# daniabib/ComfyUI_ProPainter_Nodes

Measured on NVIDIA H100. Metric: inpainted frames/sec at 640x360, 80-frame subvideo, higher is better.
Workload: dtype f16

## Files before the change

comfyui_propainter_nodes_b200/csrc/conv_epilogue.cuh:

```cuda
#pragma once
#include "conv_igemm.cuh"
#include "wgmma_ops.cuh"

namespace ppconv {

template <int ACT>
__device__ __forceinline__ void act16_t(float (&v)[16], float slope) {
#pragma unroll
  for (int i = 0; i < 16; ++i) {
    if (ACT == PP_ACT_RELU) v[i] = fmaxf(v[i], 0.f);
    else if (ACT == PP_ACT_LRELU) v[i] = v[i] > 0.f ? v[i] : v[i] * slope;
    else if (ACT == PP_ACT_SIGMOID) v[i] = ppx::sigmoidf_(v[i]);
    else if (ACT == PP_ACT_TANH) v[i] = tanhf(v[i]);
    else if (ACT == PP_ACT_GELU) v[i] = ppx::gelu_erf(v[i]);
  }
}
__device__ __forceinline__ void act16(float (&v)[16], int act, float slope) {
  switch (act) {
    case PP_ACT_RELU: act16_t<PP_ACT_RELU>(v, slope); break;
    case PP_ACT_LRELU: act16_t<PP_ACT_LRELU>(v, slope); break;
    case PP_ACT_SIGMOID: act16_t<PP_ACT_SIGMOID>(v, slope); break;
    case PP_ACT_TANH: act16_t<PP_ACT_TANH>(v, slope); break;
    case PP_ACT_GELU: act16_t<PP_ACT_GELU>(v, slope); break;
    default: break;
// ... 3 lines not shown
__device__ __forceinline__ void load16(const __half* src, int nvalid, bool vec, float (&r)[16]) {
  if (vec && nvalid == 16) {
    const uint4 a = reinterpret_cast<const uint4*>(src)[0], b = reinterpret_cast<const uint4*>(src)[1];
    const __half2* ha = reinterpret_cast<const __half2*>(&a);
    const __half2* hb = reinterpret_cast<const __half2*>(&b);
#pragma unroll
    for (int i = 0; i < 4; ++i) {
      const float2 fa = __half22float2(ha[i]), fb = __half22float2(hb[i]);
      r[2 * i] = fa.x; r[2 * i + 1] = fa.y; r[8 + 2 * i] = fb.x; r[8 + 2 * i + 1] = fb.y;
    }
  } else {
#pragma unroll
    for (int i = 0; i < 16; ++i) r[i] = i < nvalid ? __half2float(src[i]) : 0.f;
  }
}
__device__ __forceinline__ void store16(__half* dst, int nvalid, bool vec, const float (&v)[16]) {
  if (vec && nvalid == 16) {
    __align__(16) __half2 h[8];
#pragma unroll
    for (int i = 0; i < 8; ++i) h[i] = __floats2half2_rn(v[2 * i], v[2 * i + 1]);
    reinterpret_cast<uint4*>(dst)[0] = reinterpret_cast<uint4*>(h)[0];
    reinterpret_cast<uint4*>(dst)[1] = reinterpret_cast<uint4*>(h)[1];
  } else {
#pragma unroll
    for (int i = 0; i < 16; ++i)
      if (i < nvalid) dst[i] = __float2half_rn(v[i]);
  }
}

__device__ __forceinline__ void unpack16(const uint4& a, const uint4& b, float (&r)[16]) {
  const __half2* ha = reinterpret_cast<const __half2*>(&a);
  const __half2* hb = reinterpret_cast<const __half2*>(&b);
#pragma unroll
  for (int i = 0; i < 4; ++i) {
    const float2 fa = __half22float2(ha[i]), fb = __half22float2(hb[i]);
    r[2 * i] = fa.x; r[2 * i + 1] = fa.y; r[8 + 2 * i] = fb.x; r[8 + 2 * i + 1] = fb.y;
  }
// ... 16 lines not shown
    if (ng0 >= half_c) s0 = p.aux0 + mrow * p.aux0_cstride + p.aux0_coff + (ng0 - half_c);
  } else {
    s0 = p.aux0 + mrow * p.aux0_cstride + p.aux0_coff + ng0;
    s1 = p.aux1 + mrow * p.aux1_cstride + p.aux1_coff + ng0;
  }
  if (s0 == nullptr) return;
  x.have = true;
  x.a0[0] = reinterpret_cast<const uint4*>(s0)[0];
  x.a0[1] = reinterpret_cast<const uint4*>(s0)[1];
  if (s1 != nullptr) {
    x.a1[0] = reinterpret_cast<const uint4*>(s1)[0];
    x.a1[1] = reinterpret_cast<const uint4*>(s1)[1];
  }
}

__device__ __forceinline__ void conv_epilogue16(const PPConvParams& p, const uint32_t (&raw)[16], long long mrow, int g,
                                                int ng0, int epi, bool vec, const EpiAux* pre = nullptr,
                                                uint4* sm0 = nullptr, uint4* sm1 = nullptr) {
    const int nvalid = min(16, p.Cout_g - ng0);
    float v[16];
#pragma unroll
    for (int i = 0; i < 16; ++i) v[i] = __uint_as_float(raw[i]);
    if (p.bias != nullptr) {
      const float* bp = p.bias + g * p.Cout_g + ng0;
      if (vec && nvalid == 16) {
#pragma unroll
        for (int i = 0; i < 4; ++i) {
          const float4 b4 = __ldg(reinterpret_cast<const float4*>(bp) + i);
          v[4 * i] += b4.x; v[4 * i + 1] += b4.y; v[4 * i + 2] += b4.z; v[4 * i + 3] += b4.w;
        }
// ... 24 lines not shown
#pragma unroll
          for (int i = 0; i < 4; ++i)
            reinterpret_cast<float4*>(dst)[i] = make_float4(v[4 * i], v[4 * i + 1], v[4 * i + 2], v[4 * i + 3]);
        } else {
#pragma unroll
          for (int i = 0; i < 16; ++i)
            if (i < nvalid) dst[i] = v[i];
        }
      } else if (sm0 != nullptr) {
        __align__(16) __half2 h[8];
#pragma unroll
        for (int i = 0; i < 8; ++i) h[i] = __floats2half2_rn(v[2 * i], v[2 * i + 1]);
        *sm0 = reinterpret_cast<uint4*>(h)[0];
        *sm1 = reinterpret_cast<uint4*>(h)[1];
      } else {
        store16(reinterpret_cast<__half*>(p.out) + o, nvalid, vec, v);
      }
    } else if (epi == PP_EPI_GRU_ZR) {
      const int half_c = p.Cout_g >> 1;
      act16_t<PP_ACT_SIGMOID>(v, 0.f);
      if (ng0 < half_c) {
        store16(reinterpret_cast<__half*>(p.out) + mrow * p.out_cstride + p.out_coff + ng0, nvalid, vec, v);
      } else {
        const int c = ng0 - half_c;
        float h[16];
        if (pre != nullptr && pre->have) unpack16(pre->a0[0], pre->a0[1], h);
        else load16(p.aux0 + mrow * p.aux0_cstride + p.aux0_coff + c, nvalid, vec, h);
#pragma unroll
        for (int i = 0; i < 16; ++i) v[i] *= h[i];
        store16(p.out2 + mrow * p.out2_cstride + p.out2_coff + c, nvalid, vec, v);
      }
    } else {
      float h[16], z[16];
      if (pre != nullptr && pre->have) {
        unpack16(pre->a0[0], pre->a0[1], h);
        unpack16(pre->a1[0], pre->a1[1], z);
      } else {
        load16(p.aux0 + mrow * p.aux0_cstride + p.aux0_coff + ng0, nvalid, vec, h);
        load16(p.aux1 + mrow * p.aux1_cstride + p.aux1_coff + ng0, nvalid, vec, z);
      }
      act16_t<PP_ACT_TANH>(v, 0.f);
#pragma unroll
      for (int i = 0; i < 16; ++i) v[i] = (1.f - z[i]) * h[i] + z[i] * v[i];
      store16(reinterpret_cast<__half*>(p.out) + mrow * p.out_cstride + p.out_coff + ng0, nvalid, vec, v);
    }
}

constexpr int STG_LD = 40;
constexpr int STG_BYTES = 64 * STG_LD * 4;

template <int N, class Emit>
__device__ __forceinline__ void drain_acc(const float (&acc)[N / 2], float* stg, int t128, int bar_id, Emit&& emit) {
  const int wrow = 16 * (t128 >> 5) + ((t128 & 31) >> 2), wcol = 2 * (t128 & 3);
#pragma unroll 1
  for (int c0 = 0; c0 < N; c0 += 32) {
#pragma unroll
    for (int cc = 0; cc < N; cc += 32) {
      if (cc == c0) {
#pragma unroll
// ... 1 lines not shown
          if (cc + 8 * j < N) {
            const int i = (cc / 8 + j) * 4;
            *reinterpret_cast<float2*>(stg + wrow * STG_LD + 8 * j + wcol) = make_float2(acc[i], acc[i + 1]);
            *reinterpret_cast<float2*>(stg + (wrow + 8) * STG_LD + 8 * j + wcol) = make_float2(acc[i + 2], acc[i + 3]);
          }
        }
      }
    }
    ppx::named_bar(bar_id, 128);
    const int c = c0 + 16 * (t128 & 1);
    if (c < N) emit(stg + (t128 >> 1) * STG_LD + 16 * (t128 & 1), t128 >> 1, c);
    ppx::named_bar(bar_id, 128);
  }
}

__device__ __forceinline__ void epilogue_from_stage(const PPConvParams& p, const float* src, long long mrow, int g, int ng0,
                                                    uint4* sm0, uint4* sm1) {
  uint32_t raw[16];
#pragma unroll
  for (int i = 0; i < 16; i += 4) {
    const float4 v = *reinterpret_cast<const float4*>(src + i);
    raw[i] = __float_as_uint(v.x); raw[i + 1] = __float_as_uint(v.y);
    raw[i + 2] = __float_as_uint(v.z); raw[i + 3] = __float_as_uint(v.w);
  }
  conv_epilogue16(p, raw, mrow, g, ng0, p.epi, p.vec_ok != 0, nullptr, sm0, sm1);
}

template <int V>
struct IntC { static constexpr int value = V; };
template <int MAX_N, class F>
__device__ __forceinline__ void with_tile_width(int bn, F&& f) {
  switch (bn) {
    case 16: f(IntC<16>{}); break;
    case 32: f(IntC<32>{}); break;
    case 48: f(IntC<48>{}); break;
    case 64: f(IntC<64>{}); break;
    case 80: f(IntC<80>{}); break;
    case 96: f(IntC<96>{}); break;
    case 112: f(IntC<112>{}); break;
    case 128: f(IntC<128>{}); break;
// ... 21 lines not shown
```

comfyui_propainter_nodes_b200/csrc/conv_halo.cu:

```cuda
#include <cuda.h>
#include <stdlib.h>
#include <string.h>

#include <memory>

#include "conv_epilogue.cuh"
#include "conv_igemm.cuh"
#include "dcn_sample.cuh"

namespace {

constexpr int NUM_THREADS = 384;
constexpr int NUM_EPI_THREADS = 256;
constexpr int WARP_A = 8, WARP_B = 9;
constexpr int UPS_THREADS = 416, UPS_INTERP_THREADS = 128;
constexpr int UPS_WARP_B = 12;
constexpr int MAX_SA = 4, MAX_SB = 8;
constexpr int SMEM_BUDGET = 186 * 1024;

struct HaloParams {
  PPConvParams c;
  CUtensorMap tmap[4];
  int MT;
  int BW, BH;
  int tiles_x, tiles_y, n_tiles;
  int a_stage_bytes, b_stage_bytes, SA, SB;
  int tps;
  int chunks;
  int flat;
  int n_img;
  int sub_bytes;
  int ups;
  int LH, LW;
  int LBW, LBH;
  int l_stage_bytes;
  int debug;
  int tstore;
  int out_stage_bytes;
  CUtensorMap tmap_out;
};

__device__ __forceinline__ void tma_load_4d(uint32_t dst, const void* tmap, int c0, int c1, int c2, int c3, uint64_t* bar) {
  asm volatile(
      "cp.async.bulk.tensor.4d.shared::cluster.global.mbarrier::complete_tx::bytes [%0], [%1, {%3, %4, %5, %6}], [%2];" ::"r"(dst),
      "l"(tmap), "r"(ppx::smem_u32(bar)), "r"(c0), "r"(c1), "r"(c2), "r"(c3)
      : "memory");
// ... 11 lines not shown
  TileCoord t;
  t.n_idx = tile % h.n_tiles;
  int r = tile / h.n_tiles;
  t.tx = r % h.tiles_x; r /= h.tiles_x;
  t.ty = r % h.tiles_y; r /= h.tiles_y;
  t.img = r % h.n_img;
  t.g = r / h.n_img;
  return t;
}

struct Ring {
  int s;
  uint32_t ph;
};

__host__ __device__ constexpr int halo_max_tps(int bn) { return 128 / bn > 1 ? 128 / bn : 1; }

template <int BN, int MB>
__device__ __forceinline__ void halo_tap(float (&acc)[MB][BN / 2], uint64_t (&adesc)[MB], uint64_t& bdesc, uint32_t& accum,
                                         int& kx, int kw, uint32_t step_x, uint32_t step_row, uint32_t tap16) {
#pragma unroll
  for (int k = 0; k < 4; ++k)
#pragma unroll
    for (int b = 0; b < MB; ++b) ppx::wgmma_f16<BN>(acc[b], adesc[b] + 2 * k, bdesc + 2 * k, (accum | k) != 0 ? 1u : 0u);
  accum = 1u;
  bdesc += tap16;
  const uint32_t step = ++kx == kw ? step_row : step_x;
  if (kx == kw) kx = 0;
#pragma unroll
  for (int b = 0; b < MB; ++b) adesc[b] += step;
}
// ... 9 lines not shown
    wgmma_commit();
  } else {
    if constexpr (NT > 1) {
      if (tn < NT) {
        halo_tap_group<BN, MB, NT - 1>(tn, acc, adesc, bdesc, accum, kx, kw, step_x, step_row, tap16);
        return;
      }
    }
    wgmma_fence();
#pragma unroll
    for (int tt = 0; tt < NT; ++tt) halo_tap<BN, MB>(acc, adesc, bdesc, accum, kx, kw, step_x, step_row, tap16);
    wgmma_commit();
  }
}

template <int BN, int MB, int NT>
__device__ __forceinline__ void halo_tile(const HaloParams& h, int tile, uint8_t* smem, uint8_t* smem_b, int SA, int SB,
                                          int a_stage_bytes, int b_stage_bytes, uint64_t* a_full, uint64_t* a_empty,
                                          uint64_t* b_full, uint64_t* b_empty, Ring& ra, Ring& rb, float* stg,
                                          uint8_t* stg_out, int wg, int t128) {
  using namespace ppx;
  const PPConvParams& p = h.c;
  const int taps = p.kh * p.kw;
  const TileCoord t = decode_tile(h, tile);
  const int n0 = t.n_idx * p.BN;
  const int bnt = min(p.BN, p.Cout_g_pad - n0);
  const uint32_t sbo = h.flat ? 1024u : (uint32_t)h.BW * 128;
  const uint32_t step_x = (uint32_t)p.dw * 8;
  const uint32_t step_row = (uint32_t)(p.dh * h.BW - (p.kw - 1) * p.dw) * 8;
  const uint32_t tap16 = (uint32_t)p.BN * 8;
  const int kw = p.kw;
  uint32_t aoff[MB];
#pragma unroll
  for (int b = 0; b < MB; ++b) aoff[b] = MB == 2 ? wg * h.sub_bytes + b * 8 * sbo : wg * 8 * sbo;
  float acc[MB][BN / 2];
  uint32_t accum = 0;
  int pend_a = -1, pend_b = -1;
  for (int c = 0; c < h.chunks; ++c) {
    mbar_wait(&a_full[ra.s], ra.ph);
    uint64_t adesc[MB];
#pragma unroll
    for (int b = 0; b < MB; ++b) adesc[b] = gmma_desc_sw128_kmajor(smem_u32(smem + ra.s * a_stage_bytes) + aoff[b], sbo);
    int kx = 0;
    for (int tap0 = 0; tap0 < taps; tap0 += h.tps) {
      mbar_wait(&b_full[rb.s], rb.ph);
      const uint64_t bdesc = gmma_desc_sw128_kmajor(smem_u32(smem_b + rb.s * b_stage_bytes));
      halo_tap_group<BN, MB, NT>(min(h.tps, taps - tap0), acc, adesc, bdesc, accum, kx, kw, step_x, step_row, tap16);
      wgmma_wait<1>();
      if (pend_b >= 0) mbar_arrive(&b_empty[pend_b]);
      if (pend_a >= 0) mbar_arrive(&a_empty[pend_a]);
      pend_b = rb.s;
      pend_a = tap0 + h.tps >= taps ? ra.s : -1;
      if (++rb.s == SB) { rb.s = 0; rb.ph ^= 1; }
    }
    if (++ra.s == SA) { ra.s = 0; ra.ph ^= 1; }
  }
  wgmma_wait<0>();
#pragma unroll
  for (int b = 0; b < MB; ++b) wgmma_fence_acc(acc[b]);
  if (pend_b >= 0) mbar_arrive(&b_empty[pend_b]);
  if (pend_a >= 0) mbar_arrive(&a_empty[pend_a]);

  const bool skip = (h.debug & 1) != 0;
  const int bar_id = 2 + (MB == 2 ? wg : 0), bar_n = MB == 2 ? 128 : 256;
  const bool issuer = t128 == 0 && (MB == 2 || wg == 0);
  uint8_t* so = h.tstore ? stg_out + (MB == 2 ? wg : 0) * h.out_stage_bytes : nullptr;
  if (so != nullptr) {
    if (issuer) asm volatile("cp.async.bulk.wait_group.read 0;" ::: "memory");
    named_bar(bar_id, bar_n);
  }
#pragma unroll
  for (int b = 0; b < MB; ++b) {
    const int sub = MB == 2 ? wg : 0, rbase = MB == 2 ? 64 * b : 64 * wg;
    ppconv::drain_acc<BN>(acc[b], stg, t128, 4 + wg, [&](const float* src, int r64, int cc) {
      const int r = rbase + r64;
      bool mvalid;
      long long mrow;
      if (h.flat) {
        mrow = ((long long)t.tx * h.MT + sub) * 128 + r;
        mvalid = mrow < p.M_total;
      } else {
        const int oy = t.ty * 16 + (r >> 3), ox = t.tx * (8 * h.MT) + 8 * sub + (r & 7);
        mvalid = oy < p.OH && ox < p.OW;
        mrow = ((long long)t.img * p.OH + oy) * p.OW + ox;
      }
      if (!mvalid || skip || cc >= bnt || n0 + cc >= p.Cout_g) return;
      if (so != nullptr) {
        auto slot = [&](int u) {
          const int unit = ((cc & 63) >> 3) + u;
          return reinterpret_cast<uint4*>(so + (cc >> 6) * 16384 + r * 128 + ((unit ^ (r & 7)) << 4));
        };
        ppconv::epilogue_from_stage(p, src, mrow, t.g, n0 + cc, slot(0), slot(1));
      } else {
        ppconv::epilogue_from_stage(p, src, mrow, t.g, n0 + cc, nullptr, nullptr);
      }
    });
  }
  if (so != nullptr) {
    fence_proxy_async();
    named_bar(bar_id, bar_n);
    if (issuer && !skip) {
      const int row0 = (int)(((long long)t.tx * h.MT + (MB == 2 ? wg : 0)) * 128);
      for (int pnl = 0; pnl * 64 < bnt; ++pnl)
        tma_store_2d(&h.tmap_out, smem_u32(so + pnl * 16384), n0 + pnl * 64, row0);
      asm volatile("cp.async.bulk.commit_group;" ::: "memory");
    }
  }
}

template <class F>
__device__ __forceinline__ void with_tile_shape(int mt, int bn, F&& f) {
  if (mt == 2) ppconv::with_tile_width<128>(bn, [&](auto n) { f(n, ppconv::IntC<2>{}); });
  else ppconv::with_tile_width<256>(bn, [&](auto n) { f(n, ppconv::IntC<1>{}); });
}

template <bool UPS>
__global__ void __launch_bounds__(UPS ? UPS_THREADS : NUM_THREADS, 1) conv_halo_kernel(const __grid_constant__ HaloParams h) {
  using namespace ppx;
  const PPConvParams& p = h.c;
  extern __shared__ uint8_t smem_raw[];
  const uint32_t raw_addr = smem_u32(smem_raw);
  uint8_t* smem = smem_raw + (((raw_addr + 1023u) & ~1023u) - raw_addr);
  uint8_t* smem_b = smem + h.SA * h.a_stage_bytes;
  uint64_t* a_full = reinterpret_cast<uint64_t*>(smem_b + h.SB * h.b_stage_bytes);
  uint64_t* a_empty = a_full + MAX_SA;
  uint64_t* b_full = a_empty + MAX_SA;
  uint64_t* b_empty = b_full + MAX_SB;
  uint64_t* l_full = b_empty + MAX_SB;
  uint64_t* l_empty = l_full + 2;
  uint8_t* stg_out = smem_b + h.SB * h.b_stage_bytes + 2048;
  float* acc_stg = reinterpret_cast<float*>(smem_b + h.SB * h.b_stage_bytes + 1024 + (UPS ? 2 * h.l_stage_bytes : 0) +
                                            (h.tstore ? 1024 + h.MT * h.out_stage_bytes : 0));
  constexpr int W_B = UPS ? UPS_WARP_B : WARP_B;

  const int tid = threadIdx.x, warp = tid >> 5;
  const int total_tiles = h.n_tiles * h.tiles_x * h.tiles_y * h.n_img * p.groups;
  const int taps = p.kh * p.kw;

  if (tid == 0) {
    for (int s = 0; s < h.SA; ++s) { mbar_init(&a_full[s], UPS ? UPS_INTERP_THREADS : 1); mbar_init(&a_empty[s], NUM_EPI_THREADS); }
    if (UPS) for (int s = 0; s < 2; ++s) { mbar_init(&l_full[s], 1); mbar_init(&l_empty[s], UPS_INTERP_THREADS); }
    for (int s = 0; s < h.SB; ++s) { mbar_init(&b_full[s], 1); mbar_init(&b_empty[s], NUM_EPI_THREADS); }
    mbar_fence_init();
  }
  __syncthreads();
  asm volatile("griddepcontrol.wait;" ::: "memory");
  asm volatile("griddepcontrol.launch_dependents;" ::: "memory");

  if constexpr (!UPS) {
    if (warp < 8) setmaxnreg_inc<232>();
    else setmaxnreg_dec<40>();
  }
  if (warp < 8) {
    const int wg = tid >> 7, t128 = tid & 127;
    float* stg = acc_stg + wg * (ppconv::STG_BYTES / 4);
    Ring ra = {0, 0}, rb = {0, 0};
    auto run = [&](auto bn, auto mb) {
      constexpr int BN = decltype(bn)::value;
      for (int tile = blockIdx.x; tile < total_tiles; tile += gridDim.x)
        halo_tile<BN, decltype(mb)::value, halo_max_tps(BN)>(h, tile, smem, smem_b, h.SA, h.SB, h.a_stage_bytes, h.b_stage_bytes,
                                                             a_full, a_empty, b_full, b_empty, ra, rb, stg, stg_out, wg, t128);
    };
    if constexpr (UPS) ppconv::with_tile_width<128>(p.BN, [&](auto bn) { run(bn, ppconv::IntC<1>{}); });
    else with_tile_shape(h.MT, p.BN, run);
    if (h.tstore) asm volatile("cp.async.bulk.wait_group 0;" ::: "memory");
  } else if (UPS && warp < 12) {
    const int it_id = tid - 256;
    uint8_t* stg = smem_b + h.SB * h.b_stage_bytes + 1024;
    const float sy = (float)(h.LH - 1) / (float)(2 * h.LH - 1), sx = (float)(h.LW - 1) / (float)(2 * h.LW - 1);
    const uint32_t lbytes = (uint32_t)(h.LBW * h.LBH * 128);
    const bool issuer = warp == 8 && elect_one();
    auto low_origin = [&](const TileCoord& t, int& xlo, int& ylo) {
      const int X0 = t.tx * (8 * h.MT) - p.pw, Y0 = t.ty * 16 - p.ph;
      xlo = (int)(sx * (float)max(X0, 0));
      ylo = (int)(sy * (float)max(Y0, 0));
    };
    auto issue = [&](int tile, int c, int ls, uint32_t lph) {
      const TileCoord t = decode_tile(h, tile);
      int xlo, ylo;
      low_origin(t, xlo, ylo);
      mbar_wait(&l_empty[ls], lph ^ 1);
      mbar_arrive_expect_tx(&l_full[ls], lbytes);
      tma_load_4d(smem_u32(stg + ls * h.l_stage_bytes), &h.tmap[0], c * 64, xlo, ylo, t.img, &l_full[ls]);
    };
    int ls = 0, sa = 0;
    uint32_t lph = 0, pa = 0;
    int is_ls = 0;
    uint32_t is_ph = 0;
    if (issuer && blockIdx.x < total_tiles) {
      issue(blockIdx.x, 0, is_ls, is_ph);
      if (++is_ls == 2) { is_ls = 0; is_ph ^= 1; }
    }
    for (int tile = blockIdx.x; tile < total_tiles; tile += gridDim.x) {
      const TileCoord t = decode_tile(h, tile);
      const int X0 = t.tx * (8 * h.MT) - p.pw, Y0 = t.ty * 16 - p.ph;
      int xlo, ylo;
      low_origin(t, xlo, ylo);
      for (int c = 0; c < h.chunks; ++c) {
        if (issuer) {
          int nt = tile, nc = c + 1;
          if (nc == h.chunks) { nc = 0; nt += gridDim.x; }
          if (nt < total_tiles) {
            issue(nt, nc, is_ls, is_ph);
            if (++is_ls == 2) { is_ls = 0; is_ph ^= 1; }
          }
        }
        __syncwarp();
        mbar_wait(&l_full[ls], lph);
        mbar_wait(&a_empty[sa], pa ^ 1);
        const uint8_t* src = stg + ls * h.l_stage_bytes;
        uint8_t* dstA = smem + sa * h.a_stage_bytes;
        const int items = h.BW * h.BH * 8;
        for (int item = it_id; item < items; item += UPS_INTERP_THREADS) {
          const int ch = item & 7, pp = item >> 3;
          const int py = pp / h.BW, px = pp - py * h.BW;
          const int Y = Y0 + py, X = X0 + px;
// ... 23 lines not shown
          }
          *reinterpret_cast<uint4*>(dstA + pp * 128 + ((ch ^ (pp & 7)) << 4)) = o;
        }
        fence_proxy_async();
        mbar_arrive(&a_full[sa]);
        mbar_arrive(&l_empty[ls]);
        if (++ls == 2) { ls = 0; lph ^= 1; }
        if (++sa == h.SA) { sa = 0; pa ^= 1; }
      }
    }
  } else if (!UPS && warp == WARP_A) {
    if (ppx::elect_one()) {
      int s = 0;
      uint32_t phase = 0;
      const uint32_t bytes = (uint32_t)(h.BW * h.BH * 128);
      for (int tile = blockIdx.x; tile < total_tiles; tile += gridDim.x) {
        const TileCoord t = decode_tile(h, tile);
        const int x0 = h.flat ? t.tx * (128 * h.MT) : t.tx * (8 * h.MT) - p.pw, y0 = h.flat ? 0 : t.ty * 16 - p.ph;
        for (int c = 0; c < h.chunks; ++c) {
          const int ci = c * 64;
          int q = 0;
#pragma unroll
          for (int k = 1; k < 4; ++k)
            if (k < p.nseg && ci >= p.seg[k].cbegin) q = k;
          const int ch0 = t.g * p.seg[q].gstep + (ci - p.seg[q].cbegin);
          mbar_wait(&a_empty[s], phase ^ 1);
          mbar_arrive_expect_tx(&a_full[s], bytes);
          tma_load_4d(smem_u32(smem + s * h.a_stage_bytes), &h.tmap[q], ch0, x0, y0, t.img, &a_full[s]);
          if (++s == h.SA) { s = 0; phase ^= 1; }
        }
      }
    }
  } else if (warp == W_B) {
    if (ppx::elect_one()) {
      int s = 0;
      uint32_t phase = 0;
      for (int tile = blockIdx.x; tile < total_tiles; tile += gridDim.x) {
        const TileCoord t = decode_tile(h, tile);
        const int n0 = t.n_idx * p.BN;
        const uint32_t bytes = (uint32_t)(min(p.BN, p.Cout_g_pad - n0) * 128);
        const __half* wbase = p.wpacked + ((long long)t.g * p.num_kc * p.Cout_g_pad + n0) * 64;
        for (int c = 0; c < h.chunks; ++c) {
          for (int tap0 = 0; tap0 < taps; tap0 += h.tps) {
            const int tn = min(h.tps, taps - tap0);
            mbar_wait(&b_empty[s], phase ^ 1);
            mbar_arrive_expect_tx(&b_full[s], bytes * (uint32_t)tn);
            for (int t = 0; t < tn; ++t) {
              const int kc = (tap0 + t) * h.chunks + c;
              bulk_g2s(smem_u32(smem_b + s * h.b_stage_bytes + t * p.BN * 128), wbase + (long long)kc * p.Cout_g_pad * 64, bytes,
                       &b_full[s]);
            }
            if (++s == h.SB) { s = 0; phase ^= 1; }
          }
        }
      }
    }
  }
}

constexpr int PROG_MAX_LAYERS = 10;
enum { PROG_CONV = 0, PROG_DCN = 1 };

struct ProgParams {
  int n_layers;
  int SA, SB, a_stage_bytes, b_stage_bytes;
  unsigned int* counter;
  unsigned int base;
  unsigned long long* ts;
  int kind[PROG_MAX_LAYERS];
  PPDcnArgs dcn[PROG_MAX_LAYERS];
  HaloParams layer[PROG_MAX_LAYERS];
};
// ... 207 lines not shown

int halo_num_sms(int* out) {
  static int num_sms = 0;
  if (num_sms == 0) {
    int dev = 0;
    PP_CUDA_CHECK(cudaGetDevice(&dev));
    PP_CUDA_CHECK(cudaDeviceGetAttribute(&num_sms, cudaDevAttrMultiProcessorCount, dev));
    PP_CUDA_CHECK(cudaFuncSetAttribute(conv_halo_kernel<false>, cudaFuncAttributeMaxDynamicSharedMemorySize, 224 * 1024));
    PP_CUDA_CHECK(cudaFuncSetAttribute(conv_halo_kernel<true>, cudaFuncAttributeMaxDynamicSharedMemorySize, 224 * 1024));
    PP_CUDA_CHECK(cudaFuncSetAttribute(conv_prog_kernel, cudaFuncAttributeMaxDynamicSharedMemorySize, 224 * 1024));
  }
  *out = num_sms;
  return PP_OK;
}

int halo_configure(const PPConvParams& pin, HaloParams& h, bool one_wave) {
  h.c = pin;
  PPConvParams& p = h.c;
  int num_sms = 0;
  PP_TRY(halo_num_sms(&num_sms));
  const bool flat = p.kh * p.kw == 1;
  const int n_tiles0 = pp_ceil_div(p.Cout_g_pad, 128);
  int bn = pp_ceil_div(pp_ceil_div(p.Cout_g_pad, n_tiles0), 16) * 16;
  const int tiles_y = flat ? 1 : pp_ceil_div(p.OH, 16);
  auto tiles_x = [&](int mt) { return flat ? (int)pp_ceil_div64(p.M_total, 128 * mt) : pp_ceil_div(p.OW, 8 * mt); };
  const int n_img = flat ? 1 : p.N;
  auto count = [&](int mt, int bn_) {
    return (long long)pp_ceil_div(p.Cout_g_pad, bn_) * tiles_x(mt) * tiles_y * n_img * p.groups;
  };
  int mt = 2;
  if (p.ups2x || count(2, bn) < num_sms) mt = 1;
  while (count(mt, bn) < num_sms && bn >= 64 && bn % 32 == 0) bn /= 2;
  if (one_wave && !p.ups2x) {
    mt = 1;
    static int min_bn = -1;
    if (min_bn < 0) { const char* e = getenv("PP_PROG_MIN_BN"); min_bn = e != nullptr ? atoi(e) : 16; }
    for (int nt = 8; nt >= 1; --nt) {
      const int b = pp_ceil_div(pp_ceil_div(p.Cout_g_pad, nt), 16) * 16;
      if (b > 128 || b < 16 || (b < min_bn && nt > 1)) continue;
      if (count(1, b) <= num_sms) { mt = 1; bn = b; break; }
    }
  }
  p.BN = bn;
  h.MT = mt;
  h.flat = flat ? 1 : 0;
  h.n_img = n_img;
  h.BW = flat ? 128 * mt : 8 * mt + (p.kw - 1) * p.dw;
  h.BH = flat ? 1 : 16 + (p.kh - 1) * p.dh;
  h.sub_bytes = flat ? 128 * 128 : 8 * 128;
  h.tiles_x = tiles_x(mt);
  h.tiles_y = tiles_y;
  h.n_tiles = pp_ceil_div(p.Cout_g_pad, bn);
  h.chunks = pp_ceil_div(p.Cin, 64);
  h.a_stage_bytes = pp_ceil_div(h.BW * h.BH * 128, 1024) * 1024;
  {
    static int max_tps = -1;
    if (max_tps < 0) { const char* e = getenv("PP_HALO_TPS"); max_tps = e != nullptr ? atoi(e) : 9; }
    int tps = halo_max_tps(bn);
    if (tps > p.kh * p.kw) tps = p.kh * p.kw;
    if (tps > max_tps) tps = max_tps;
    if (tps < 1 || p.ups2x) tps = 1;
    h.tps = tps;
  }
  h.b_stage_bytes = h.tps * bn * 128;
  h.ups = p.ups2x ? 1 : 0;
  h.LH = p.H / 2; h.LW = p.W / 2;
  h.LBW = (h.BW - 1) / 2 + 3; h.LBH = (h.BH - 1) / 2 + 3;
  h.l_stage_bytes = h.ups ? pp_ceil_div(h.LBW * h.LBH * 128, 1024) * 1024 : 0;
  h.tstore = 0;
  h.out_stage_bytes = 0;
  {
    static int ts_on = -1;
    if (ts_on < 0) { const char* e = getenv("PP_TMA_STORE"); ts_on = (e == nullptr || atoi(e) != 0) ? 1 : 0; }
// ... 68 lines not shown

inline long long halo_total_tiles(const HaloParams& h) {
  return (long long)h.n_tiles * h.tiles_x * h.tiles_y * h.n_img * h.c.groups;
}

}

int pp_launch_conv_halo(const PPConvParams& pin, cudaStream_t stream) {
  HaloParams h;
  PP_TRY(halo_configure(pin, h, false));
  int num_sms = 0;
  PP_TRY(halo_num_sms(&num_sms));
  const long long total_tiles = halo_total_tiles(h);
  const size_t smem = (size_t)h.SA * h.a_stage_bytes + (size_t)h.SB * h.b_stage_bytes + 1024 + 1024 + 2 * (size_t)h.l_stage_bytes +
                      (h.tstore ? (size_t)h.MT * h.out_stage_bytes + 1024 : 0) + 2 * ppconv::STG_BYTES;
  const int grid = (int)(total_tiles < num_sms ? total_tiles : num_sms);
  cudaLaunchConfig_t cfg;
  memset(&cfg, 0, sizeof(cfg));
  cfg.gridDim = dim3(grid);
  cfg.blockDim = dim3(h.ups ? UPS_THREADS : NUM_THREADS);
  cfg.dynamicSmemBytes = smem;
  cfg.stream = stream;
  cudaLaunchAttribute attr[1];
  attr[0].id = cudaLaunchAttributeProgrammaticStreamSerialization;
  attr[0].val.programmaticStreamSerializationAllowed = 1;
  cfg.attrs = attr;
  cfg.numAttrs = 1;
  if (h.ups) PP_CUDA_CHECK(cudaLaunchKernelEx(&cfg, conv_halo_kernel<true>, h));
  else PP_CUDA_CHECK(cudaLaunchKernelEx(&cfg, conv_halo_kernel<false>, h));
  PP_CUDA_CHECK(cudaGetLastError());
  return PP_OK;
}

namespace {
thread_local PPProgRecorder* g_recorder = nullptr;
}

struct PPProgRecorder {
  ProgParams prog;
  double flops = 0.0;
  int n_conv = 0;
};
// ... 111 lines not shown
```

comfyui_propainter_nodes_b200/csrc/pp_common.cuh:

```cuda
#pragma once
#include <cuda_runtime.h>
#include <cuda_fp16.h>
#include <stdint.h>
#include <stdio.h>

#define PP_OK 0
#define PP_ERR_CUDA 1
#define PP_ERR_ARG 2
#define PP_ERR_STATE 3

void pp_set_error(const char* fmt, ...);

#define PP_CUDA_CHECK(expr)                                                                   \
  do {                                                                                        \
    cudaError_t _e = (expr);                                                                  \
    if (_e != cudaSuccess) {                                                                  \
      pp_set_error("%s:%d CUDA error %s: %s", __FILE__, __LINE__, #expr, cudaGetErrorString(_e)); \
      return PP_ERR_CUDA;                                                                     \
    }                                                                                         \
  } while (0)

#define PP_REQUIRE(cond, ...)        \
  do {                               \
    if (!(cond)) {                   \
// ... 96 lines not shown
}
__device__ __forceinline__ void cp_async_commit() { asm volatile("cp.async.commit_group;" ::: "memory"); }
template <int N>
__device__ __forceinline__ void cp_async_wait() {
  asm volatile("cp.async.wait_group %0;" ::"n"(N) : "memory");
}
__device__ __forceinline__ void fence_proxy_async() { asm volatile("fence.proxy.async.shared::cta;" ::: "memory"); }

__device__ __forceinline__ void bulk_g2s(uint32_t dst_smem, const void* src, uint32_t bytes, uint64_t* bar) {
  asm volatile(
      "cp.async.bulk.shared::cluster.global.mbarrier::complete_tx::bytes [%0], [%1], %2, [%3];" ::"r"(dst_smem),
      "l"(src), "r"(bytes), "r"(smem_u32(bar))
      : "memory");
}

__device__ __forceinline__ void wgmma_fence() { asm volatile("wgmma.fence.sync.aligned;" ::: "memory"); }
__device__ __forceinline__ void wgmma_commit() { asm volatile("wgmma.commit_group.sync.aligned;" ::: "memory"); }
template <int N>
__device__ __forceinline__ void wgmma_wait() {
  asm volatile("wgmma.wait_group.sync.aligned %0;" ::"n"(N) : "memory");
}
template <int N>
__device__ __forceinline__ void wgmma_fence_acc(float (&d)[N]) {
#pragma unroll
  for (int i = 0; i < N; ++i) asm volatile("" : "+f"(d[i])::"memory");
}

__device__ __forceinline__ uint64_t gmma_desc_sw128(uint32_t smem_addr, uint32_t lbo, uint32_t sbo) {
  uint64_t d = 0;
  d |= (uint64_t)((smem_addr & 0x3FFFF) >> 4);
// ... 38 lines not shown
```

Measured before the change: 122.8.

## Run non-upsampling halo conv as 2-CTA clusters with multicast weights and ping-pong warpgroups

The non-upsampling halo convolution now launches as 2-CTA clusters. Each CTA loads half of every weight stage and multicasts it to both CTAs, while the two consumer warpgroups alternate whole tiles in ping-pong order and each covers 256 output rows. The weight-stage size can grow to 32 KB so more taps are grouped per stage, and a vectorised tail store path is added to the epilogue. The aim is to halve per-CTA weight traffic from global memory and to overlap one warpgroup's epilogue with the other's MMA. In exchange it adds cross-CTA barrier traffic and cluster scheduling constraints, and it may reduce occupancy through the larger shared-memory footprint.

```diff
diff --git a/comfyui_propainter_nodes_b200/csrc/conv_epilogue.cuh b/comfyui_propainter_nodes_b200/csrc/conv_epilogue.cuh
--- a/comfyui_propainter_nodes_b200/csrc/conv_epilogue.cuh
+++ b/comfyui_propainter_nodes_b200/csrc/conv_epilogue.cuh
@@ -41,6 +41,7 @@
     for (int i = 0; i < 16; ++i) r[i] = i < nvalid ? __half2float(src[i]) : 0.f;
   }
 }
+template <bool TAIL = false>
 __device__ __forceinline__ void store16(__half* dst, int nvalid, bool vec, const float (&v)[16]) {
   if (vec && nvalid == 16) {
     __align__(16) __half2 h[8];
@@ -48,6 +49,29 @@
     for (int i = 0; i < 8; ++i) h[i] = __floats2half2_rn(v[2 * i], v[2 * i + 1]);
     reinterpret_cast<uint4*>(dst)[0] = reinterpret_cast<uint4*>(h)[0];
     reinterpret_cast<uint4*>(dst)[1] = reinterpret_cast<uint4*>(h)[1];
+  } else if (TAIL && vec) {
+    uint32_t w[8];
+#pragma unroll
+    for (int i = 0; i < 8; ++i) {
+      const __half2 hh = __floats2half2_rn(v[2 * i], v[2 * i + 1]);
+      w[i] = *reinterpret_cast<const uint32_t*>(&hh);
+    }
+#pragma unroll
+    for (int j = 0; j < 2; ++j) {
+      const int n = nvalid - 8 * j;
+      __half* d = dst + 8 * j;
+      const uint32_t* q = w + 4 * j;
+      if (n >= 8) {
+        *reinterpret_cast<uint4*>(d) = make_uint4(q[0], q[1], q[2], q[3]);
+      } else if (n > 0) {
+        const int r = n & 3;
+        __half* d2 = n >= 4 ? d + 4 : d;
+        const uint32_t a = n >= 4 ? q[2] : q[0], b = n >= 4 ? q[3] : q[1];
+        if (n >= 4) *reinterpret_cast<uint2*>(d) = make_uint2(q[0], q[1]);
+        if (r >= 2) *reinterpret_cast<uint32_t*>(d2) = a;
+        if (r & 1) *reinterpret_cast<unsigned short*>(d2 + (r & 2)) = (unsigned short)((r >= 2 ? b : a) & 0xFFFFu);
+      }
+    }
   } else {
 #pragma unroll
     for (int i = 0; i < 16; ++i)
@@ -94,6 +118,7 @@
   }
 }
 
+template <bool TAIL = false>
 __device__ __forceinline__ void conv_epilogue16(const PPConvParams& p, const uint32_t (&raw)[16], long long mrow, int g,
                                                 int ng0, int epi, bool vec, const EpiAux* pre = nullptr,
                                                 uint4* sm0 = nullptr, uint4* sm1 = nullptr) {
@@ -148,13 +173,13 @@
         *sm0 = reinterpret_cast<uint4*>(h)[0];
         *sm1 = reinterpret_cast<uint4*>(h)[1];
       } else {
-        store16(reinterpret_cast<__half*>(p.out) + o, nvalid, vec, v);
+        store16<TAIL>(reinterpret_cast<__half*>(p.out) + o, nvalid, vec, v);
       }
     } else if (epi == PP_EPI_GRU_ZR) {
       const int half_c = p.Cout_g >> 1;
       act16_t<PP_ACT_SIGMOID>(v, 0.f);
       if (ng0 < half_c) {
-        store16(reinterpret_cast<__half*>(p.out) + mrow * p.out_cstride + p.out_coff + ng0, nvalid, vec, v);
+        store16<TAIL>(reinterpret_cast<__half*>(p.out) + mrow * p.out_cstride + p.out_coff + ng0, nvalid, vec, v);
       } else {
         const int c = ng0 - half_c;
         float h[16];
@@ -162,7 +187,7 @@
         else load16(p.aux0 + mrow * p.aux0_cstride + p.aux0_coff + c, nvalid, vec, h);
 #pragma unroll
         for (int i = 0; i < 16; ++i) v[i] *= h[i];
-        store16(p.out2 + mrow * p.out2_cstride + p.out2_coff + c, nvalid, vec, v);
+        store16<TAIL>(p.out2 + mrow * p.out2_cstride + p.out2_coff + c, nvalid, vec, v);
       }
     } else {
       float h[16], z[16];
@@ -176,7 +201,7 @@
       act16_t<PP_ACT_TANH>(v, 0.f);
 #pragma unroll
       for (int i = 0; i < 16; ++i) v[i] = (1.f - z[i]) * h[i] + z[i] * v[i];
-      store16(reinterpret_cast<__half*>(p.out) + mrow * p.out_cstride + p.out_coff + ng0, nvalid, vec, v);
+      store16<TAIL>(reinterpret_cast<__half*>(p.out) + mrow * p.out_cstride + p.out_coff + ng0, nvalid, vec, v);
     }
 }
 
@@ -208,6 +233,7 @@
   }
 }
 
+template <bool TAIL = false>
 __device__ __forceinline__ void epilogue_from_stage(const PPConvParams& p, const float* src, long long mrow, int g, int ng0,
                                                     uint4* sm0, uint4* sm1) {
   uint32_t raw[16];
@@ -217,7 +243,7 @@
     raw[i] = __float_as_uint(v.x); raw[i + 1] = __float_as_uint(v.y);
     raw[i + 2] = __float_as_uint(v.z); raw[i + 3] = __float_as_uint(v.w);
   }
-  conv_epilogue16(p, raw, mrow, g, ng0, p.epi, p.vec_ok != 0, nullptr, sm0, sm1);
+  conv_epilogue16<TAIL>(p, raw, mrow, g, ng0, p.epi, p.vec_ok != 0, nullptr, sm0, sm1);
 }
 
 template <int V>
diff --git a/comfyui_propainter_nodes_b200/csrc/conv_halo.cu b/comfyui_propainter_nodes_b200/csrc/conv_halo.cu
--- a/comfyui_propainter_nodes_b200/csrc/conv_halo.cu
+++ b/comfyui_propainter_nodes_b200/csrc/conv_halo.cu
@@ -29,7 +29,6 @@
   int chunks;
   int flat;
   int n_img;
-  int sub_bytes;
   int ups;
   int LH, LW;
   int LBW, LBH;
@@ -71,7 +70,10 @@
   uint32_t ph;
 };
 
-__host__ __device__ constexpr int halo_max_tps(int bn) { return 128 / bn > 1 ? 128 / bn : 1; }
+__host__ __device__ constexpr int halo_max_tps(int bn, int stage_kb = 16) {
+  return stage_kb * 8 / bn > 8 ? 8 : stage_kb * 8 / bn > 1 ? stage_kb * 8 / bn : 1;
+}
+constexpr int HALO_BIG_STAGE_KB = 32;
 
 template <int BN, int MB>
 __device__ __forceinline__ void halo_tap(float (&acc)[MB][BN / 2], uint64_t (&adesc)[MB], uint64_t& bdesc, uint32_t& accum,
@@ -111,11 +113,29 @@
   }
 }
 
+struct PingPong {
+  uint64_t* ord;
+  int k;
+  uint32_t peer_b_empty;
+};
+
+template <int MB>
+__device__ __forceinline__ void halo_release_b(uint64_t* b_empty, int s, int t128, const PingPong* pp) {
+  if constexpr (MB == 2) {
+    if ((t128 & 31) == 0) {
+      ppx::mbar_arrive(&b_empty[s]);
+      ppx::mbar_arrive_cluster(pp->peer_b_empty + s * 8);
+    }
+  } else {
+    ppx::mbar_arrive(&b_empty[s]);
+  }
+}
+
 template <int BN, int MB, int NT>
 __device__ __forceinline__ void halo_tile(const HaloParams& h, int tile, uint8_t* smem, uint8_t* smem_b, int SA, int SB,
                                           int a_stage_bytes, int b_stage_bytes, uint64_t* a_full, uint64_t* a_empty,
                                           uint64_t* b_full, uint64_t* b_empty, Ring& ra, Ring& rb, float* stg,
-                                          uint8_t* stg_out, int wg, int t128) {
+                                          uint8_t* stg_out, int wg, int t128, int sub = 0, const PingPong* pp = nullptr) {
   using namespace ppx;
   const PPConvParams& p = h.c;
   const int taps = p.kh * p.kw;
@@ -129,7 +149,12 @@
   const int kw = p.kw;
   uint32_t aoff[MB];
 #pragma unroll
-  for (int b = 0; b < MB; ++b) aoff[b] = MB == 2 ? wg * h.sub_bytes + b * 8 * sbo : wg * 8 * sbo;
+  for (int b = 0; b < MB; ++b) aoff[b] = MB == 2 ? b * 8 * sbo : wg * 8 * sbo;
+  if constexpr (MB == 2) {
+    const int j = pp->k >> 1;
+    if (wg == 1) mbar_wait(&pp->ord[1], j & 1);
+    else if (j > 0) mbar_wait(&pp->ord[0], (j - 1) & 1);
+  }
   float acc[MB][BN / 2];
   uint32_t accum = 0;
   int pend_a = -1, pend_b = -1;
@@ -144,7 +169,7 @@
       const uint64_t bdesc = gmma_desc_sw128_kmajor(smem_u32(smem_b + rb.s * b_stage_bytes));
       halo_tap_group<BN, MB, NT>(min(h.tps, taps - tap0), acc, adesc, bdesc, accum, kx, kw, step_x, step_row, tap16);
       wgmma_wait<1>();
-      if (pend_b >= 0) mbar_arrive(&b_empty[pend_b]);
+      if (pend_b >= 0) halo_release_b<MB>(b_empty, pend_b, t128, pp);
       if (pend_a >= 0) mbar_arrive(&a_empty[pend_a]);
       pend_b = rb.s;
       pend_a = tap0 + h.tps >= taps ? ra.s : -1;
@@ -152,10 +177,11 @@
     }
     if (++ra.s == SA) { ra.s = 0; ra.ph ^= 1; }
   }
+  if constexpr (MB == 2) mbar_arrive(&pp->ord[wg ^ 1]);
   wgmma_wait<0>();
 #pragma unroll
   for (int b = 0; b < MB; ++b) wgmma_fence_acc(acc[b]);
-  if (pend_b >= 0) mbar_arrive(&b_empty[pend_b]);
+  if (pend_b >= 0) halo_release_b<MB>(b_empty, pend_b, t128, pp);
   if (pend_a >= 0) mbar_arrive(&a_empty[pend_a]);
 
   const bool skip = (h.debug & 1) != 0;
@@ -168,7 +194,7 @@
   }
 #pragma unroll
   for (int b = 0; b < MB; ++b) {
-    const int sub = MB == 2 ? wg : 0, rbase = MB == 2 ? 64 * b : 64 * wg;
+    const int rbase = MB == 2 ? 64 * b : 64 * wg;
     ppconv::drain_acc<BN>(acc[b], stg, t128, 4 + wg, [&](const float* src, int r64, int cc) {
       const int r = rbase + r64;
       bool mvalid;
@@ -187,17 +213,17 @@
           const int unit = ((cc & 63) >> 3) + u;
           return reinterpret_cast<uint4*>(so + (cc >> 6) * 16384 + r * 128 + ((unit ^ (r & 7)) << 4));
         };
-        ppconv::epilogue_from_stage(p, src, mrow, t.g, n0 + cc, slot(0), slot(1));
+        ppconv::epilogue_from_stage<MB == 2>(p, src, mrow, t.g, n0 + cc, slot(0), slot(1));
       } else {
-        ppconv::epilogue_from_stage(p, src, mrow, t.g, n0 + cc, nullptr, nullptr);
+        ppconv::epilogue_from_stage<MB == 2>(p, src, mrow, t.g, n0 + cc, nullptr, nullptr);
       }
     });
   }
   if (so != nullptr) {
     fence_proxy_async();
     named_bar(bar_id, bar_n);
-    if (issuer && !skip) {
-      const int row0 = (int)(((long long)t.tx * h.MT + (MB == 2 ? wg : 0)) * 128);
+    const int row0 = (int)(((long long)t.tx * h.MT + sub) * 128);
+    if (issuer && !skip && row0 < p.M_total) {
       for (int pnl = 0; pnl * 64 < bnt; ++pnl)
         tma_store_2d(&h.tmap_out, smem_u32(so + pnl * 16384), n0 + pnl * 64, row0);
       asm volatile("cp.async.bulk.commit_group;" ::: "memory");
@@ -205,10 +231,8 @@
   }
 }
 
-template <class F>
-__device__ __forceinline__ void with_tile_shape(int mt, int bn, F&& f) {
-  if (mt == 2) ppconv::with_tile_width<128>(bn, [&](auto n) { f(n, ppconv::IntC<2>{}); });
-  else ppconv::with_tile_width<256>(bn, [&](auto n) { f(n, ppconv::IntC<1>{}); });
+__device__ __forceinline__ void ring_skip(Ring& r, int n, int S) {
+  for (r.s += n; r.s >= S; r.s -= S) r.ph ^= 1;
 }
 
 template <bool UPS>
@@ -225,6 +249,7 @@
   uint64_t* b_empty = b_full + MAX_SB;
   uint64_t* l_full = b_empty + MAX_SB;
   uint64_t* l_empty = l_full + 2;
+  uint64_t* ord = l_empty + 2;
   uint8_t* stg_out = smem_b + h.SB * h.b_stage_bytes + 2048;
   float* acc_stg = reinterpret_cast<float*>(smem_b + h.SB * h.b_stage_bytes + 1024 + (UPS ? 2 * h.l_stage_bytes : 0) +
                                             (h.tstore ? 1024 + h.MT * h.out_stage_bytes : 0));
@@ -233,14 +258,19 @@
   const int tid = threadIdx.x, warp = tid >> 5;
   const int total_tiles = h.n_tiles * h.tiles_x * h.tiles_y * h.n_img * p.groups;
   const int taps = p.kh * p.kw;
+  const int first = UPS ? blockIdx.x : blockIdx.x >> 1, step = UPS ? gridDim.x : gridDim.x >> 1;
+  const uint32_t rank = UPS ? 0u : cluster_ctarank();
 
   if (tid == 0) {
-    for (int s = 0; s < h.SA; ++s) { mbar_init(&a_full[s], UPS ? UPS_INTERP_THREADS : 1); mbar_init(&a_empty[s], NUM_EPI_THREADS); }
+    const uint32_t a_cons = UPS ? NUM_EPI_THREADS : 128, b_cons = UPS ? NUM_EPI_THREADS : 8;
+    for (int s = 0; s < h.SA; ++s) { mbar_init(&a_full[s], UPS ? UPS_INTERP_THREADS : 1); mbar_init(&a_empty[s], a_cons); }
     if (UPS) for (int s = 0; s < 2; ++s) { mbar_init(&l_full[s], 1); mbar_init(&l_empty[s], UPS_INTERP_THREADS); }
-    for (int s = 0; s < h.SB; ++s) { mbar_init(&b_full[s], 1); mbar_init(&b_empty[s], NUM_EPI_THREADS); }
+    else for (int w = 0; w < 2; ++w) mbar_init(&ord[w], 128);
+    for (int s = 0; s < h.SB; ++s) { mbar_init(&b_full[s], 1); mbar_init(&b_empty[s], b_cons); }
     mbar_fence_init();
   }
-  __syncthreads();
+  if constexpr (UPS) __syncthreads();
+  else cluster_sync();
   asm volatile("griddepcontrol.wait;" ::: "memory");
   asm volatile("griddepcontrol.launch_dependents;" ::: "memory");
 
@@ -252,14 +282,29 @@
     const int wg = tid >> 7, t128 = tid & 127;
     float* stg = acc_stg + wg * (ppconv::STG_BYTES / 4);
     Ring ra = {0, 0}, rb = {0, 0};
-    auto run = [&](auto bn, auto mb) {
-      constexpr int BN = decltype(bn)::value;
-      for (int tile = blockIdx.x; tile < total_tiles; tile += gridDim.x)
-        halo_tile<BN, decltype(mb)::value, halo_max_tps(BN)>(h, tile, smem, smem_b, h.SA, h.SB, h.a_stage_bytes, h.b_stage_bytes,
-                                                             a_full, a_empty, b_full, b_empty, ra, rb, stg, stg_out, wg, t128);
-    };
-    if constexpr (UPS) ppconv::with_tile_width<128>(p.BN, [&](auto bn) { run(bn, ppconv::IntC<1>{}); });
-    else with_tile_shape(h.MT, p.BN, run);
+    if constexpr (UPS) {
+      ppconv::with_tile_width<128>(p.BN, [&](auto bn) {
+        constexpr int BN = decltype(bn)::value;
+        for (int tile = first; tile < total_tiles; tile += step)
+          halo_tile<BN, 1, halo_max_tps(BN)>(h, tile, smem, smem_b, h.SA, h.SB, h.a_stage_bytes, h.b_stage_bytes, a_full,
+                                             a_empty, b_full, b_empty, ra, rb, stg, stg_out, wg, t128);
+      });
+    } else {
+      const int na = h.chunks, nb = h.chunks * ((taps + h.tps - 1) / h.tps);
+      PingPong pp = {ord, 0, mapa_shared(smem_u32(b_empty), rank ^ 1u)};
+      ppconv::with_tile_width<128>(p.BN, [&](auto bn) __attribute__((always_inline)) {
+        constexpr int BN = decltype(bn)::value;
+        for (int tile = first; tile < total_tiles; tile += step, ++pp.k) {
+          if ((pp.k & 1) != wg) {
+            ring_skip(ra, na, h.SA);
+            ring_skip(rb, nb, h.SB);
+            continue;
+          }
+          halo_tile<BN, 2, halo_max_tps(BN, HALO_BIG_STAGE_KB)>(h, tile, smem, smem_b, h.SA, h.SB, h.a_stage_bytes, h.b_stage_bytes, a_full,
+                                             a_empty, b_full, b_empty, ra, rb, stg, stg_out, wg, t128, (int)rank, &pp);
+        }
+      });
+    }
     if (h.tstore) asm volatile("cp.async.bulk.wait_group 0;" ::: "memory");
   } else if (UPS && warp < 12) {
     const int it_id = tid - 256;
@@ -284,11 +329,11 @@
     uint32_t lph = 0, pa = 0;
     int is_ls = 0;
     uint32_t is_ph = 0;
-    if (issuer && blockIdx.x < total_tiles) {
-      issue(blockIdx.x, 0, is_ls, is_ph);
+    if (issuer && first < total_tiles) {
+      issue(first, 0, is_ls, is_ph);
       if (++is_ls == 2) { is_ls = 0; is_ph ^= 1; }
     }
-    for (int tile = blockIdx.x; tile < total_tiles; tile += gridDim.x) {
+    for (int tile = first; tile < total_tiles; tile += step) {
       const TileCoord t = decode_tile(h, tile);
       const int X0 = t.tx * (8 * h.MT) - p.pw, Y0 = t.ty * 16 - p.ph;
       int xlo, ylo;
@@ -296,7 +341,7 @@
       for (int c = 0; c < h.chunks; ++c) {
         if (issuer) {
           int nt = tile, nc = c + 1;
-          if (nc == h.chunks) { nc = 0; nt += gridDim.x; }
+          if (nc == h.chunks) { nc = 0; nt += step; }
           if (nt < total_tiles) {
             issue(nt, nc, is_ls, is_ph);
             if (++is_ls == 2) { is_ls = 0; is_ph ^= 1; }
@@ -350,9 +395,10 @@
       int s = 0;
       uint32_t phase = 0;
       const uint32_t bytes = (uint32_t)(h.BW * h.BH * 128);
-      for (int tile = blockIdx.x; tile < total_tiles; tile += gridDim.x) {
+      for (int tile = first; tile < total_tiles; tile += step) {
         const TileCoord t = decode_tile(h, tile);
-        const int x0 = h.flat ? t.tx * (128 * h.MT) : t.tx * (8 * h.MT) - p.pw, y0 = h.flat ? 0 : t.ty * 16 - p.ph;
+        const int sx = t.tx * h.MT + (int)rank;
+        const int x0 = h.flat ? sx * 128 : sx * 8 - p.pw, y0 = h.flat ? 0 : t.ty * 16 - p.ph;
         for (int c = 0; c < h.chunks; ++c) {
           const int ci = c * 64;
           int q = 0;
@@ -371,7 +417,7 @@
     if (ppx::elect_one()) {
       int s = 0;
       uint32_t phase = 0;
-      for (int tile = blockIdx.x; tile < total_tiles; tile += gridDim.x) {
+      for (int tile = first; tile < total_tiles; tile += step) {
         const TileCoord t = decode_tile(h, tile);
         const int n0 = t.n_idx * p.BN;
         const uint32_t bytes = (uint32_t)(min(p.BN, p.Cout_g_pad - n0) * 128);
@@ -383,8 +429,14 @@
             mbar_arrive_expect_tx(&b_full[s], bytes * (uint32_t)tn);
             for (int t = 0; t < tn; ++t) {
               const int kc = (tap0 + t) * h.chunks + c;
-              bulk_g2s(smem_u32(smem_b + s * h.b_stage_bytes + t * p.BN * 128), wbase + (long long)kc * p.Cout_g_pad * 64, bytes,
-                       &b_full[s]);
+              const uint32_t dst = smem_u32(smem_b + s * h.b_stage_bytes + t * p.BN * 128);
+              const __half* src = wbase + (long long)kc * p.Cout_g_pad * 64;
+              if constexpr (UPS) {
+                bulk_g2s(dst, src, bytes, &b_full[s]);
+              } else {
+                const uint32_t half = bytes / 2;
+                bulk_g2s_multicast(dst + rank * half, reinterpret_cast<const uint8_t*>(src) + rank * half, half, &b_full[s], 0x3);
+              }
             }
             if (++s == h.SB) { s = 0; phase ^= 1; }
           }
@@ -392,6 +444,7 @@
       }
     }
   }
+  if constexpr (!UPS) cluster_sync();
 }
 
 constexpr int PROG_MAX_LAYERS = 10;
@@ -629,6 +682,30 @@
   return PP_OK;
 }
 
+int halo_max_clusters(int* out) {
+  static int max_clusters = 0;
+  if (max_clusters == 0) {
+    int num_sms = 0;
+    PP_TRY(halo_num_sms(&num_sms));
+    cudaLaunchConfig_t cfg;
+    memset(&cfg, 0, sizeof(cfg));
+    cfg.gridDim = dim3(2 * num_sms);
+    cfg.blockDim = dim3(NUM_THREADS);
+    cfg.dynamicSmemBytes = 224 * 1024;
+    cudaLaunchAttribute attr[1];
+    attr[0].id = cudaLaunchAttributeClusterDimension;
+    attr[0].val.clusterDim.x = 2;
+    attr[0].val.clusterDim.y = 1;
+    attr[0].val.clusterDim.z = 1;
+    cfg.attrs = attr;
+    cfg.numAttrs = 1;
+    PP_CUDA_CHECK(cudaOccupancyMaxActiveClusters(&max_clusters, conv_halo_kernel<false>, &cfg));
+    PP_REQUIRE(max_clusters > 0, "conv_halo: no 2-CTA cluster fits the device");
+  }
+  *out = max_clusters;
+  return PP_OK;
+}
+
 int halo_configure(const PPConvParams& pin, HaloParams& h, bool one_wave) {
   h.c = pin;
   PPConvParams& p = h.c;
@@ -643,26 +720,23 @@
   auto count = [&](int mt, int bn_) {
     return (long long)pp_ceil_div(p.Cout_g_pad, bn_) * tiles_x(mt) * tiles_y * n_img * p.groups;
   };
-  int mt = 2;
-  if (p.ups2x || count(2, bn) < num_sms) mt = 1;
+  int mt = p.ups2x || one_wave ? 1 : 2;
   while (count(mt, bn) < num_sms && bn >= 64 && bn % 32 == 0) bn /= 2;
   if (one_wave && !p.ups2x) {
-    mt = 1;
     static int min_bn = -1;
     if (min_bn < 0) { const char* e = getenv("PP_PROG_MIN_BN"); min_bn = e != nullptr ? atoi(e) : 16; }
     for (int nt = 8; nt >= 1; --nt) {
       const int b = pp_ceil_div(pp_ceil_div(p.Cout_g_pad, nt), 16) * 16;
       if (b > 128 || b < 16 || (b < min_bn && nt > 1)) continue;
-      if (count(1, b) <= num_sms) { mt = 1; bn = b; break; }
+      if (count(1, b) <= num_sms) { bn = b; break; }
     }
   }
   p.BN = bn;
   h.MT = mt;
   h.flat = flat ? 1 : 0;
   h.n_img = n_img;
-  h.BW = flat ? 128 * mt : 8 * mt + (p.kw - 1) * p.dw;
+  h.BW = flat ? 128 : 8 + (p.kw - 1) * p.dw;
   h.BH = flat ? 1 : 16 + (p.kh - 1) * p.dh;
-  h.sub_bytes = flat ? 128 * 128 : 8 * 128;
   h.tiles_x = tiles_x(mt);
   h.tiles_y = tiles_y;
   h.n_tiles = pp_ceil_div(p.Cout_g_pad, bn);
@@ -671,7 +745,8 @@
   {
     static int max_tps = -1;
     if (max_tps < 0) { const char* e = getenv("PP_HALO_TPS"); max_tps = e != nullptr ? atoi(e) : 9; }
-    int tps = halo_max_tps(bn);
+    const bool big = !one_wave && !p.ups2x && 3 * (h.a_stage_bytes + HALO_BIG_STAGE_KB * 1024) <= SMEM_BUDGET;
+    int tps = halo_max_tps(bn, big ? HALO_BIG_STAGE_KB : 16);
     if (tps > p.kh * p.kw) tps = p.kh * p.kw;
     if (tps > max_tps) tps = max_tps;
     if (tps < 1 || p.ups2x) tps = 1;
@@ -770,18 +845,27 @@
   const long long total_tiles = halo_total_tiles(h);
   const size_t smem = (size_t)h.SA * h.a_stage_bytes + (size_t)h.SB * h.b_stage_bytes + 1024 + 1024 + 2 * (size_t)h.l_stage_bytes +
                       (h.tstore ? (size_t)h.MT * h.out_stage_bytes + 1024 : 0) + 2 * ppconv::STG_BYTES;
-  const int grid = (int)(total_tiles < num_sms ? total_tiles : num_sms);
+  int grid = (int)(total_tiles < num_sms ? total_tiles : num_sms);
+  if (!h.ups) {
+    int max_clusters = 0;
+    PP_TRY(halo_max_clusters(&max_clusters));
+    grid = 2 * (int)(total_tiles < max_clusters ? total_tiles : max_clusters);
+  }
   cudaLaunchConfig_t cfg;
   memset(&cfg, 0, sizeof(cfg));
   cfg.gridDim = dim3(grid);
   cfg.blockDim = dim3(h.ups ? UPS_THREADS : NUM_THREADS);
   cfg.dynamicSmemBytes = smem;
   cfg.stream = stream;
-  cudaLaunchAttribute attr[1];
+  cudaLaunchAttribute attr[2];
   attr[0].id = cudaLaunchAttributeProgrammaticStreamSerialization;
   attr[0].val.programmaticStreamSerializationAllowed = 1;
+  attr[1].id = cudaLaunchAttributeClusterDimension;
+  attr[1].val.clusterDim.x = 2;
+  attr[1].val.clusterDim.y = 1;
+  attr[1].val.clusterDim.z = 1;
   cfg.attrs = attr;
-  cfg.numAttrs = 1;
+  cfg.numAttrs = h.ups ? 1 : 2;
   if (h.ups) PP_CUDA_CHECK(cudaLaunchKernelEx(&cfg, conv_halo_kernel<true>, h));
   else PP_CUDA_CHECK(cudaLaunchKernelEx(&cfg, conv_halo_kernel<false>, h));
   PP_CUDA_CHECK(cudaGetLastError());
diff --git a/comfyui_propainter_nodes_b200/csrc/pp_common.cuh b/comfyui_propainter_nodes_b200/csrc/pp_common.cuh
--- a/comfyui_propainter_nodes_b200/csrc/pp_common.cuh
+++ b/comfyui_propainter_nodes_b200/csrc/pp_common.cuh
@@ -134,6 +134,32 @@
       : "memory");
 }
 
+__device__ __forceinline__ void bulk_g2s_multicast(uint32_t dst_smem, const void* src, uint32_t bytes, uint64_t* bar,
+                                                   uint16_t cta_mask) {
+  asm volatile(
+      "cp.async.bulk.shared::cluster.global.mbarrier::complete_tx::bytes.multicast::cluster [%0], [%1], %2, [%3], %4;" ::"r"(
+          dst_smem),
+      "l"(src), "r"(bytes), "r"(smem_u32(bar)), "h"(cta_mask)
+      : "memory");
+}
+
+__device__ __forceinline__ uint32_t cluster_ctarank() {
+  uint32_t r;
+  asm volatile("mov.u32 %0, %%cluster_ctarank;" : "=r"(r));
+  return r;
+}
+__device__ __forceinline__ uint32_t mapa_shared(uint32_t smem_addr, uint32_t rank) {
+  uint32_t r;
+  asm volatile("mapa.shared::cluster.u32 %0, %1, %2;" : "=r"(r) : "r"(smem_addr), "r"(rank));
+  return r;
+}
+__device__ __forceinline__ void mbar_arrive_cluster(uint32_t cluster_addr) {
+  asm volatile("mbarrier.arrive.shared::cluster.b64 _, [%0];" ::"r"(cluster_addr) : "memory");
+}
+__device__ __forceinline__ void cluster_sync() {
+  asm volatile("barrier.cluster.arrive.release;\n\tbarrier.cluster.wait.acquire;" ::: "memory");
+}
+
 __device__ __forceinline__ void wgmma_fence() { asm volatile("wgmma.fence.sync.aligned;" ::: "memory"); }
 __device__ __forceinline__ void wgmma_commit() { asm volatile("wgmma.commit_group.sync.aligned;" ::: "memory"); }
 template <int N>
```

Result: faster. 125.1, median of 6 (+1.9%).
